# kakao/buffalo

Measured on NVIDIA H100. Metric: interactions/sec (nnz/s) ALS d=128, higher is better.
Workload: dtype f32

## Files before the change

buffalo_b200/csrc/als_tc.cuh:

```cuda
#pragma once
#include "als_generic.cuh"
#include "bfl_common.cuh"
#include <type_traits>

#include "sm90_ptx.cuh"

namespace bfl {
namespace tc {

using namespace sm90;

constexpr int N_CONV = 4, KH = N_CONV / 4;
constexpr int W_EPI = 0, W_MMA = 4, W_CONV = 8, W_PLAN = W_CONV + N_CONV;
constexpr int WARPS = 16, THREADS = WARPS * 32;
constexpr int REG_MMA = 200, REG_PLAN = 4 * 128 - 128 - 128 - REG_MMA;
constexpr int NXS = 8;
constexpr int PT = 2;
constexpr int NR = 2;
constexpr int NO = 2;
constexpr int GATHER_AHEAD = 1;
constexpr int NPG = 8, NP = NPG * PT;
constexpr int NBV = 8;
template <int D>
struct Cfg {
    static constexpr int TILE = D == 128 ? 32 : 16;
    static constexpr int NF = D / 128;
    static constexpr int LBO = D * 16;
    static constexpr int OP_BYTES = TILE * D * 2;
};
constexpr uint32_t F_FIRST = 1u << 8, F_LAST = 1u << 9, F_NEG = 1u << 10, F_STOP = 1u << 11;

__device__ __forceinline__ int msw(int c) { return ((c >> 1) & 3) << 3; }

template <int D>
struct Smem {
    static constexpr int TILE = Cfg<D>::TILE;
    alignas(1024) unsigned char op[NO][PT][2][Cfg<D>::OP_BYTES];
    alignas(128) float raw[NR][PT][TILE * D];
    alignas(128) float mat[128 * 128];
    alignas(16) float bvec[NBV][KH][D];
    alignas(16) float sumq[NBV][KH][D];
    alignas(16) float xs[NXS][D];
    alignas(16) float pv[4][32];
    alignas(16) float dl[4][32];
    alignas(16) float sws[NP][TILE];
    alignas(16) float wv[NP][TILE];
    alignas(16) int32_t keys[NP][TILE];
    float wsum[NBV][KH];
    uint32_t meta_raw[NP];
    uint32_t meta_op[NO][PT];
    int badrow[NXS];
    alignas(8) uint64_t plan_full[NPG], plan_empty[NPG], raw_full[NR], raw_empty[NR], op_full[NO], op_empty[NO];
    alignas(8) uint64_t acc_full, acc_empty, x_full[NXS], d_full[4];
};

struct TcArgs {
    AlsArgs a;
    const int32_t* items;
    float* scratch;
    int64_t split;
    int pass;
    int debug;
};

template <int D>
__host__ __device__ constexpr size_t scratch_floats() { return (size_t)D * D + 2 * D + 4; }

__global__ void tc_absmax_kernel(const float* __restrict__ p, size_t n, unsigned int* __restrict__ out) {
    float m = 0.f;
    const size_t gtid = (size_t)blockIdx.x * blockDim.x + threadIdx.x, gsz = (size_t)gridDim.x * blockDim.x;
    const size_t lead = min(n, (size_t)(((16 - ((uintptr_t)p & 15)) & 15) / 4));
    const size_t n4 = (n - lead) / 4;
    const float4* p4 = reinterpret_cast<const float4*>(p + lead);
    for (size_t i = gtid; i < n4; i += gsz) {
        const float4 v = __ldg(p4 + i);
        m = fmaxf(fmaxf(m, fmaxf(fabsf(v.x), fabsf(v.y))), fmaxf(fabsf(v.z), fabsf(v.w)));
    }
    for (size_t i = gtid; i < lead; i += gsz) m = fmaxf(m, fabsf(p[i]));
    for (size_t i = lead + n4 * 4 + gtid; i < n; i += gsz) m = fmaxf(m, fabsf(p[i]));
    for (int o = 16; o > 0; o >>= 1) m = fmaxf(m, __shfl_xor_sync(FULL, m, o));
    if ((threadIdx.x & 31) == 0 && m > 0.f) atomicMax(out, __float_as_uint(m));
}
__global__ void tc_scale_kernel(const unsigned int* __restrict__ ymax, const unsigned int* __restrict__ vmax, float alpha,
                                float* __restrict__ out) {
    const float y = __uint_as_float(*ymax), w = __uint_as_float(*vmax) * fabsf(alpha);
    const float top = y * sqrtf(w);
    int e = 0;
    if (top > 0.f && isfinite(top)) {
        int ex;
        frexpf(top, &ex);
        e = 15 - ex;
    }
    e = max(-60, min(60, e));
    out[0] = ldexpf(1.f, e);
    out[1] = ldexpf(1.f, -2 * e);
}

template <int D, bool PARTIAL, bool LOSS1>
__global__ void __launch_bounds__(THREADS, 1) als_tc_kernel(TcArgs ta) {
    static_assert(D == 128 || (D == 256 && PARTIAL), "fused row solve: d = 128; split-row mode: d = 128 or 256");
    constexpr int TILE = Cfg<D>::TILE, NF = Cfg<D>::NF, LBO = Cfg<D>::LBO;
    extern __shared__ __align__(1024) unsigned char smem_raw_[];
    Smem<D>& S = *reinterpret_cast<Smem<D>*>(smem_raw_);
    const AlsArgs& a = ta.a;
    const int tid = threadIdx.x, lane = tid & 31;
    const int warp = __shfl_sync(FULL, tid >> 5, 0);

    if (tid == 0) {
        for (int i = 0; i < NR; ++i) {
            mbar_init(&S.raw_full[i], N_CONV);
            mbar_init(&S.raw_empty[i], N_CONV);
        }
        for (int i = 0; i < NPG; ++i) {
            mbar_init(&S.plan_full[i], 1);
            mbar_init(&S.plan_empty[i], N_CONV);
        }
        for (int i = 0; i < NO; ++i) {
            mbar_init(&S.op_full[i], N_CONV);
            mbar_init(&S.op_empty[i], 4);
        }
        mbar_init(&S.acc_full, 4);
        mbar_init(&S.acc_empty, 4);
        for (int b = 0; b < 4; ++b) mbar_init(&S.d_full[b], 1);
        for (int i = 0; i < NXS; ++i) {
            mbar_init(&S.x_full[i], 4);
            S.badrow[i] = 0;
        }
        mbar_init_fence();
    }
    __syncthreads();
    const float scale = __ldg(a.tc_scales), inv2 = __ldg(a.tc_scales + 1);

    const int64_t nitems = a.row_end - a.row_begin;
    const int64_t my_first = (int64_t)blockIdx.x;
    const int64_t stride = gridDim.x;

    auto item_info = [&](int64_t it, int& row, int64_t& beg, int64_t& n, int& slot) {
        if (PARTIAL) {
            const int32_t* p = ta.items + 3 * (a.row_begin + it);
            row = p[0];
            const int64_t rb = row == 0 ? 0 : a.indptr[row - 1];
            const int64_t rn = a.indptr[row] - rb;
            beg = rb + (int64_t)p[1] * ta.split;
            n = min(ta.split, rn - (int64_t)p[1] * ta.split);
            slot = p[2];
        } else {
            row = a.row_list[a.row_begin + it];
            beg = row == 0 ? 0 : a.indptr[row - 1];
            n = a.indptr[row] - beg;
            slot = 0;
        }
    };

    if (warp >= W_PLAN) {
        setmaxnreg_dec<REG_PLAN>();
        if (warp != W_PLAN) return;
        uint32_t gsl = 0, rph = 0, pe = 0;
        auto tile_begin = [&]() -> uint32_t {
            if (pe == 0) mbar_wait_idle(&S.plan_empty[gsl], rph ^ 1u);
            return gsl * PT + pe;
        };
        auto tile_end = [&]() {
            if (++pe == PT) {
                if (lane == 0) mbar_arrive(&S.plan_full[gsl]);
                pe = 0;
                if (++gsl == NPG) { gsl = 0; rph ^= 1u; }
            }
        };
        auto emit = [&](unsigned mask, uint32_t flags, int32_t key, float w) {
            const int cnt = __popc(mask);
            const int slot = __popc(mask & ((1u << lane) - 1u));
            const uint32_t rs = tile_begin();
            if ((mask >> lane) & 1u) {
                S.keys[rs][slot] = key;
                S.sws[rs][slot] = sqrtf(fabsf(w)) * scale;
                S.wv[rs][slot] = w;
            } else {
                const int zslot = cnt + lane - slot;
                if (zslot < TILE) {
                    S.sws[rs][zslot] = 0.f;
                    S.wv[rs][zslot] = 0.f;
                }
            }
            if (lane == 0) S.meta_raw[rs] = (uint32_t)cnt | flags;
            __syncwarp();
            tile_end();
        };
        constexpr int SC = 4, SCN = SC * TILE;
        const bool inl = lane < TILE;
        auto load_id = [&](int64_t it, int& row, int& chunk) {
            row = -1;
            chunk = 0;
            if (it < nitems) {
                if (PARTIAL) {
                    const int32_t* p = ta.items + 3 * (a.row_begin + it);
                    row = p[0];
                    chunk = p[1];
                } else {
                    row = a.row_list[a.row_begin + it];
                }
            }
        };
        auto load_span = [&](int row, int chunk, const int32_t*& kp, const float*& vp, int& n) {
            kp = a.keys;
            vp = a.vals;
            n = 0;
            if (row >= 0) {
                const int64_t rb = row == 0 ? 0 : a.indptr[row - 1];
                const int64_t rn = a.indptr[row] - rb;
                int64_t beg = rb;
                n = (int)rn;
                if (PARTIAL) {
                    beg = rb + (int64_t)chunk * ta.split;
                    n = (int)min(ta.split, rn - (int64_t)chunk * ta.split);
                }
                kp = a.keys + (beg - a.shift);
                vp = a.vals + (beg - a.shift);
            }
        };
        auto load_sc = [&](const int32_t* kp, const float* vp, int n, int c0, int32_t (&key)[SC], float (&w)[SC]) {
#pragma unroll
            for (int s = 0; s < SC; ++s) {
                const int idx = c0 + s * TILE + lane;
                const bool ok = inl && idx < n;
                key[s] = ok ? kp[idx] : 0;
                w[s] = ok ? vp[idx] * a.alpha : 0.f;
            }
        };
        auto emit_sc = [&](int n, int c0, const int32_t (&key)[SC], const float (&w)[SC]) {
            bool neg = false;
#pragma unroll
            for (int s = 0; s < SC; ++s) neg |= w[s] < 0.f;
            if (!__any_sync(FULL, neg)) {
#pragma unroll
                for (int s = 0; s < SC; ++s) {
                    const int t0 = c0 + s * TILE;
                    if (t0 < n) {
                        const uint32_t meta = (uint32_t)min(TILE, n - t0) | (t0 == 0 ? F_FIRST : 0u) | (t0 + TILE >= n ? F_LAST : 0u);
                        const uint32_t rs = tile_begin();
                        if (inl) {
                            float sq;
                            asm("sqrt.approx.ftz.f32 %0, %1;" : "=f"(sq) : "f"(w[s]));
                            S.keys[rs][lane] = key[s];
                            S.sws[rs][lane] = sq * scale;
                            S.wv[rs][lane] = w[s];
                        }
                        if (lane == 0) S.meta_raw[rs] = meta;
                        __syncwarp();
                        tile_end();
                    }
                }
            } else {
#pragma unroll
                for (int s = 0; s < SC; ++s) {
                    const int t0 = c0 + s * TILE;
                    if (t0 < n) {
                        const bool valid = inl && t0 + lane < n;
                        const unsigned pm = __ballot_sync(FULL, valid && !(w[s] < 0.f));
                        const unsigned nm = __ballot_sync(FULL, valid && (w[s] < 0.f));
                        const bool lastc = t0 + TILE >= n;
                        uint32_t fl = (t0 == 0 ? F_FIRST : 0u);
                        if (pm) {
                            emit(pm, fl | ((lastc && !nm) ? F_LAST : 0u), key[s], w[s]);
                            fl = 0u;
                        }
                        if (nm) emit(nm, fl | F_NEG | (lastc ? F_LAST : 0u), key[s], w[s]);
                    }
                }
            }
        };
        const int32_t *kp0, *kp1, *kp2, *kp3;
        const float *vp0, *vp1, *vp2, *vp3;
        int n0, n1, n2, n3;
        int row_t, ch_t, row4, ch4;
        int32_t k0[SC], k1[SC], k2[SC], nk[SC];
        float w0[SC], w1[SC], w2[SC], nw[SC];
        load_id(my_first, row_t, ch_t);
        load_span(row_t, ch_t, kp0, vp0, n0);
        load_sc(kp0, vp0, n0, 0, k0, w0);
        load_id(my_first + stride, row_t, ch_t);
        load_span(row_t, ch_t, kp1, vp1, n1);
        load_sc(kp1, vp1, n1, 0, k1, w1);
        load_id(my_first + 2 * stride, row_t, ch_t);
        load_span(row_t, ch_t, kp2, vp2, n2);
        load_id(my_first + 3 * stride, row4, ch4);
        for (int64_t it = my_first; it < nitems; it += stride) {
            load_sc(kp2, vp2, n2, 0, k2, w2);
            load_span(row4, ch4, kp3, vp3, n3);
            load_id(it + 4 * stride, row4, ch4);
            for (int c0 = 0; c0 < n0; c0 += SCN) {
                const bool more = c0 + SCN < n0;
                if (more) load_sc(kp0, vp0, n0, c0 + SCN, nk, nw);
                emit_sc(n0, c0, k0, w0);
                if (more) {
#pragma unroll
                    for (int s = 0; s < SC; ++s) { k0[s] = nk[s]; w0[s] = nw[s]; }
                }
            }
#pragma unroll
            for (int s = 0; s < SC; ++s) { k0[s] = k1[s]; w0[s] = w1[s]; k1[s] = k2[s]; w1[s] = w2[s]; }
            kp0 = kp1; vp0 = vp1; n0 = n1; kp1 = kp2; vp1 = vp2; n1 = n2; kp2 = kp3; vp2 = vp3; n2 = n3;
        }
        do {
            const uint32_t rs = tile_begin();
            if (lane == 0) S.meta_raw[rs] = F_STOP;
            __syncwarp();
            tile_end();
        } while (pe != 0);
    } else if (warp >= W_MMA && warp < W_MMA + 4) {
        setmaxnreg_inc<REG_MMA>();
        const int r0 = (D == 256 && ta.pass == 2) ? 128 : 0, c0 = (D == 256 && ta.pass > 0) ? 128 : 0;
        const int wq = warp - W_MMA;
        const int fr = 16 * wq + (lane >> 2), fc = 2 * (lane & 3);
        float d0[64], d1[64];
        auto acc_init = [&]() {
            const float s2 = scale * scale;
#pragma unroll
            for (int n = 0; n < 16; ++n)
#pragma unroll
                for (int h = 0; h < 2; ++h) {
                    const int r = fr + 8 * h, c = 8 * n + fc;
                    float2 g0 = make_float2(0.f, 0.f), g1 = make_float2(0.f, 0.f);
                    if (!PARTIAL) {
                        g0 = __ldg(reinterpret_cast<const float2*>(a.G + (size_t)r * D + c));
                        g1 = __ldg(reinterpret_cast<const float2*>(a.G + (size_t)(r + 64) * D + c));
                        g0.x += r == c ? a.reg : 0.f;
                        g0.y += r == c + 1 ? a.reg : 0.f;
                        g1.x += r + 64 == c ? a.reg : 0.f;
                        g1.y += r + 64 == c + 1 ? a.reg : 0.f;
                    }
                    d0[4 * n + 2 * h] = g0.x * s2; d0[4 * n + 2 * h + 1] = g0.y * s2;
                    d1[4 * n + 2 * h] = g1.x * s2; d1[4 * n + 2 * h + 1] = g1.y * s2;
                }
        };
        uint32_t os = 0, oph = 0, aph = 0;
        int64_t seq = 0;
        bool stop = false;
        acc_init();
        while (!stop) {
            mbar_wait(&S.op_full[os], oph);
            fence_proxy_async_smem();
#pragma unroll 1
            for (int e = 0; e < PT; ++e) {
                const uint32_t meta = S.meta_op[os][e];
                if (meta & F_STOP) {
                    stop = true;
                    break;
                }
                const int ksteps = (ta.debug & 2) ? 0 : (int)(meta & 0xffu);
                const uint32_t hi = s32(&S.op[os][e][0][0]), lo = s32(&S.op[os][e][1][0]);
                wgmma_fence();
#pragma unroll 1
                for (int ks = 0; ks < ksteps; ++ks) {
                    const uint32_t k0 = ks * 2 * LBO;
                    const uint64_t ah0 = smem_desc(hi + k0 + r0 * 16, LBO, 128), ah1 = smem_desc(hi + k0 + (r0 + 64) * 16, LBO, 128);
                    const uint64_t al0 = smem_desc(lo + k0 + r0 * 16, LBO, 128), al1 = smem_desc(lo + k0 + (r0 + 64) * 16, LBO, 128);
                    const uint64_t bh = smem_desc(hi + k0 + c0 * 16, LBO, 128), bl = smem_desc(lo + k0 + c0 * 16, LBO, 128);
                    if (meta & F_NEG) {
                        wgmma_m64n128k16_f16<true>(d0, ah0, bh);
                        wgmma_m64n128k16_f16<true>(d0, ah0, bl);
                        wgmma_m64n128k16_f16<true>(d0, al0, bh);
                        wgmma_m64n128k16_f16<true>(d1, ah1, bh);
                        wgmma_m64n128k16_f16<true>(d1, ah1, bl);
                        wgmma_m64n128k16_f16<true>(d1, al1, bh);
                    } else {
                        wgmma_m64n128k16_f16<false>(d0, ah0, bh);
                        wgmma_m64n128k16_f16<false>(d0, ah0, bl);
                        wgmma_m64n128k16_f16<false>(d0, al0, bh);
                        wgmma_m64n128k16_f16<false>(d1, ah1, bh);
                        wgmma_m64n128k16_f16<false>(d1, ah1, bl);
                        wgmma_m64n128k16_f16<false>(d1, al1, bh);
                    }
                }
                wgmma_commit();
                if (meta & F_LAST) {
                    wgmma_wait<0>();
#pragma unroll
                    for (int i = 0; i < 64; ++i) { acc_fence(d0[i]); acc_fence(d1[i]); }
                    mbar_wait_idle(&S.acc_empty, aph ^ 1u);
                    if (PARTIAL) {
                        const int slot = ta.items[3 * (a.row_begin + my_first + seq * stride) + 2];
                        float* sc = ta.scratch + (size_t)slot * scratch_floats<D>();
#pragma unroll
                        for (int n = 0; n < 16; ++n)
#pragma unroll
                            for (int h = 0; h < 2; ++h)
#pragma unroll
                                for (int i = 0; i < 2; ++i) {
                                    const int r = r0 + fr + 8 * h, c = c0 + 8 * n + fc + i;
                                    const float v0 = d0[4 * n + 2 * h + i] * inv2, v1 = d1[4 * n + 2 * h + i] * inv2;
                                    atomicAdd(sc + (size_t)r * D + c, v0);
                                    atomicAdd(sc + (size_t)(r + 64) * D + c, v1);
                                    if (r0 != c0) {
                                        atomicAdd(sc + (size_t)c * D + r, v0);
                                        atomicAdd(sc + (size_t)c * D + r + 64, v1);
                                    }
                                }
                    } else {
#pragma unroll
                        for (int n = 0; n < 16; ++n)
#pragma unroll
                            for (int h = 0; h < 2; ++h)
#pragma unroll
                                for (int i = 0; i < 2; ++i) {
                                    const int r = fr + 8 * h, c = 8 * n + fc + i;
                                    S.mat[c * 128 + (r ^ msw(c))] = d0[4 * n + 2 * h + i] * inv2;
                                    S.mat[c * 128 + ((r + 64) ^ msw(c))] = d1[4 * n + 2 * h + i] * inv2;
                                }
                    }
                    __syncwarp();
                    if (lane == 0) mbar_arrive(&S.acc_full);
                    aph ^= 1u;
                    ++seq;
                    acc_init();
                }
            }
            wgmma_wait<0>();
#pragma unroll
            for (int i = 0; i < 64; ++i) { acc_fence(d0[i]); acc_fence(d1[i]); }
            __syncwarp();
            if (lane == 0) mbar_arrive(&S.op_empty[os]);
            if (++os == NO) { os = 0; oph ^= 1u; }
        }
    } else if (warp >= W_CONV && warp < W_CONV + N_CONV) {
        const int cta = tid - W_CONV * 32;
        const int ct = cta & 127;
        const int kh = cta >> 7;
        constexpr int CHS = TILE / 8 / KH;
        uint32_t rs = 0, rph = 0, os = 0, oph = 0, bslot = 0;
        float2 bacc[NF], qacc[NF];
        float wacc = 0.f;
#pragma unroll
        for (int f = 0; f < NF; ++f) { bacc[f] = make_float2(0.f, 0.f); qacc[f] = make_float2(0.f, 0.f); }
        const int cw = cta >> 5;
        uint32_t gs = 0, gph = 0, grs = 0, grph = 0;
        bool plan_end = false;
        auto gather = [&]() {
            if (plan_end) {
                cp_async_commit();
                return;
            }
            mbar_wait(&S.plan_full[gs], gph);
            mbar_wait(&S.raw_empty[grs], grph ^ 1u);
            const uint32_t gm0 = S.meta_raw[gs * PT], gm1 = S.meta_raw[gs * PT + 1];
            if (PT == 2 && !(ta.debug & 1) && ((gm0 | gm1) & F_STOP) == 0 && (gm0 & 0xffu) == TILE && (gm1 & 0xffu) == TILE) {
                int32_t kk[PT][TILE / N_CONV];
#pragma unroll
                for (int e = 0; e < PT; ++e)
#pragma unroll
                    for (int i = 0; i < TILE / N_CONV; ++i) kk[e][i] = S.keys[gs * PT + e][cw + N_CONV * i];
#pragma unroll
                for (int e = 0; e < PT; ++e)
#pragma unroll
                    for (int i = 0; i < TILE / N_CONV; ++i) {
                        const float* src = a.Y + (int64_t)kk[e][i] * a.ld + lane * 4;
                        float* dst = &S.raw[grs][e][(cw + N_CONV * i) * D + lane * 4];
#pragma unroll
                        for (int c = 0; c < D / 128; ++c) cp_async16_cg(dst + c * 128, src + c * 128);
                    }
            } else
#pragma unroll
            for (int e = 0; e < PT; ++e) {
                const uint32_t gmeta = S.meta_raw[gs * PT + e];
                if (gmeta & F_STOP) {
                    plan_end = true;
                } else {
                    const int gcnt = (ta.debug & 1) ? 0 : (int)(gmeta & 0xffu);
#pragma unroll
                    for (int i = 0; i < TILE / N_CONV; ++i) {
                        const int slot = cw + N_CONV * i;
                        if (slot < gcnt) {
                            const float* src = a.Y + (int64_t)S.keys[gs * PT + e][slot] * a.ld + lane * 4;
                            float* dst = &S.raw[grs][e][slot * D + lane * 4];
#pragma unroll
                            for (int c = 0; c < D / 128; ++c) cp_async16_cg(dst + c * 128, src + c * 128);
                        }
                    }
                }
            }
            cp_async_commit();
            if (++gs == NPG) { gs = 0; gph ^= 1u; }
            if (++grs == NR) { grs = 0; grph ^= 1u; }
        };
        uint32_t cs = 0;
        bool done = false;
        if (ta.debug & 16) {
            uint32_t ph = 0;
            for (;;) {
                mbar_wait(&S.plan_full[cs], ph);
                const bool stop = (S.meta_raw[cs * PT] | S.meta_raw[cs * PT + 1]) & F_STOP;
                __syncwarp();
                if (lane == 0) mbar_arrive(&S.plan_empty[cs]);
                if (stop) break;
                if (++cs == NPG) { cs = 0; ph ^= 1u; }
            }
            if (cta == 0) S.meta_op[0][0] = F_STOP;
            __syncwarp();
            if (lane == 0) mbar_arrive(&S.op_full[0]);
            done = true;
        }
#pragma unroll 1
        for (int i = 0; i < GATHER_AHEAD && !done; ++i) gather();
        while (!done) {
            gather();
            cp_async_wait_group<GATHER_AHEAD>();
            __syncwarp();
            if (lane == 0) mbar_arrive(&S.raw_full[rs]);
            mbar_wait(&S.raw_full[rs], rph);
            float qv[PT][CHS * 8 * NF];
#pragma unroll
            for (int e = 0; e < PT; ++e)
#pragma unroll
                for (int c = 0; c < CHS; ++c)
#pragma unroll
                    for (int i = 0; i < 8; ++i)
#pragma unroll
                        for (int f = 0; f < NF; ++f)
                            qv[e][(c * 8 + i) * NF + f] = S.raw[rs][e][((kh * CHS + c) * 8 + i) * D + ct + 128 * f];
            mbar_wait(&S.op_empty[os], oph ^ 1u);
            const uint32_t cm0 = S.meta_raw[cs * PT], cm1 = S.meta_raw[cs * PT + 1];
            const bool fast2 = PT == 2 && !(ta.debug & 4) && ((cm0 | cm1) & F_STOP) == 0 && (cm0 & 0xffu) == TILE &&
                               (cm1 & 0xffu) == TILE;
            if (fast2) {
#pragma unroll
                for (int e = 0; e < PT; ++e) {
                    const uint32_t meta = e == 0 ? cm0 : cm1;
                    const uint32_t psl = cs * PT + e;
                    const bool first = (meta & F_FIRST) != 0;
#pragma unroll
                    for (int f = 0; f < NF; ++f) {
                        bacc[f].x = first ? 0.f : bacc[f].x; bacc[f].y = first ? 0.f : bacc[f].y;
                        qacc[f].x = first ? 0.f : qacc[f].x; qacc[f].y = first ? 0.f : qacc[f].y;
                    }
                    wacc = first ? 0.f : wacc;
                    unsigned char* hi = &S.op[os][e][0][0];
                    unsigned char* lo = &S.op[os][e][1][0];
#pragma unroll
                    for (int c = 0; c < CHS; ++c) {
                        const int kc = kh * CHS + c, k0 = kc * 8;
                        const float4 sa = *reinterpret_cast<const float4*>(&S.sws[psl][k0]);
                        const float4 sb = *reinterpret_cast<const float4*>(&S.sws[psl][k0 + 4]);
                        const float4 wa = *reinterpret_cast<const float4*>(&S.wv[psl][k0]);
                        const float4 wb = *reinterpret_cast<const float4*>(&S.wv[psl][k0 + 4]);
                        if (LOSS1) wacc += ((wa.x + wa.y) + (wa.z + wa.w)) + ((wb.x + wb.y) + (wb.z + wb.w));
#pragma unroll
                        for (int f = 0; f < NF; ++f) {
                            const int m = ct + 128 * f;
                            const float* q = &qv[e][0];
                            const float2 q01 = make_float2(q[(c * 8 + 0) * NF + f], q[(c * 8 + 1) * NF + f]);
                            const float2 q23 = make_float2(q[(c * 8 + 2) * NF + f], q[(c * 8 + 3) * NF + f]);
                            const float2 q45 = make_float2(q[(c * 8 + 4) * NF + f], q[(c * 8 + 5) * NF + f]);
                            const float2 q67 = make_float2(q[(c * 8 + 6) * NF + f], q[(c * 8 + 7) * NF + f]);
                            uint4 h4, l4;
                            split_f16x2(f2mul(q01, make_float2(sa.x, sa.y)), h4.x, l4.x);
                            split_f16x2(f2mul(q23, make_float2(sa.z, sa.w)), h4.y, l4.y);
                            split_f16x2(f2mul(q45, make_float2(sb.x, sb.y)), h4.z, l4.z);
                            split_f16x2(f2mul(q67, make_float2(sb.z, sb.w)), h4.w, l4.w);
                            const int off = kc * LBO + (m >> 3) * 128 + (m & 7) * 16;
                            *reinterpret_cast<uint4*>(hi + off) = h4;
                            *reinterpret_cast<uint4*>(lo + off) = l4;
                            bacc[f] = f2fma(make_float2(wa.x, wa.y), q01, bacc[f]);
                            bacc[f] = f2fma(make_float2(wa.z, wa.w), q23, bacc[f]);
                            bacc[f] = f2fma(make_float2(wb.x, wb.y), q45, bacc[f]);
                            bacc[f] = f2fma(make_float2(wb.z, wb.w), q67, bacc[f]);
                            if (LOSS1) {
                                qacc[f].x += (q01.x + q23.x) + (q45.x + q67.x);
                                qacc[f].y += (q01.y + q23.y) + (q45.y + q67.y);
                            }
                        }
                    }
#pragma unroll
                    for (int f = 0; f < NF; ++f) {
                        S.bvec[bslot][kh][ct + 128 * f] = bacc[f].x + bacc[f].y;
                        if (LOSS1) S.sumq[bslot][kh][ct + 128 * f] = qacc[f].x + qacc[f].y;
                    }
                    if (LOSS1 && ct == 0) S.wsum[bslot][kh] = wacc;
                    bslot = (bslot + ((meta & F_LAST) ? 1u : 0u)) & (NBV - 1);
                    if (cta == 0) S.meta_op[os][e] = (uint32_t)(TILE / 16) | (meta & (F_FIRST | F_LAST | F_NEG));
                }
            } else
#pragma unroll
            for (int e = 0; e < PT; ++e) {
                if (done) continue;
                const uint32_t psl = cs * PT + e;
                const uint32_t meta = S.meta_raw[psl];
                if (meta & F_STOP) {
                    if (cta == 0) S.meta_op[os][e] = F_STOP;
                    done = true;
                    continue;
                }
                const int cnt = (int)(meta & 0xffu), ksteps = (cnt + 15) >> 4;
                if (meta & F_FIRST) {
#pragma unroll
                    for (int f = 0; f < NF; ++f) { bacc[f] = make_float2(0.f, 0.f); qacc[f] = make_float2(0.f, 0.f); }
                    wacc = 0.f;
                }
                unsigned char* hi = &S.op[os][e][0][0];
                unsigned char* lo = &S.op[os][e][1][0];
                auto chunk = [&](auto guard, const int c) {
                    constexpr bool GUARD = decltype(guard)::value;
                    const int kc = kh * CHS + c, k0 = kc * 8;
                    const float4 sa = *reinterpret_cast<const float4*>(&S.sws[psl][k0]);
                    const float4 sb = *reinterpret_cast<const float4*>(&S.sws[psl][k0 + 4]);
                    const float4 wa = *reinterpret_cast<const float4*>(&S.wv[psl][k0]);
                    const float4 wb = *reinterpret_cast<const float4*>(&S.wv[psl][k0 + 4]);
                    if (LOSS1) wacc += ((wa.x + wa.y) + (wa.z + wa.w)) + ((wb.x + wb.y) + (wb.z + wb.w));
#pragma unroll
                    for (int f = 0; f < NF; ++f) {
                        const int m = ct + 128 * f;
                        float q[8];
#pragma unroll
                        for (int i = 0; i < 8; ++i) q[i] = qv[e][(c * 8 + i) * NF + f];
                        if (GUARD) {
#pragma unroll
                            for (int i = 0; i < 8; ++i) q[i] = (k0 + i < cnt) ? q[i] : 0.f;
                        }
                        const float2 q01 = make_float2(q[0], q[1]), q23 = make_float2(q[2], q[3]);
                        const float2 q45 = make_float2(q[4], q[5]), q67 = make_float2(q[6], q[7]);
                        uint4 h4, l4;
                        split_f16x2(f2mul(q01, make_float2(sa.x, sa.y)), h4.x, l4.x);
                        split_f16x2(f2mul(q23, make_float2(sa.z, sa.w)), h4.y, l4.y);
                        split_f16x2(f2mul(q45, make_float2(sb.x, sb.y)), h4.z, l4.z);
                        split_f16x2(f2mul(q67, make_float2(sb.z, sb.w)), h4.w, l4.w);
                        const int off = kc * LBO + (m >> 3) * 128 + (m & 7) * 16;
                        *reinterpret_cast<uint4*>(hi + off) = h4;
                        *reinterpret_cast<uint4*>(lo + off) = l4;
                        bacc[f] = f2fma(make_float2(wa.x, wa.y), q01, bacc[f]);
                        bacc[f] = f2fma(make_float2(wa.z, wa.w), q23, bacc[f]);
                        bacc[f] = f2fma(make_float2(wb.x, wb.y), q45, bacc[f]);
                        bacc[f] = f2fma(make_float2(wb.z, wb.w), q67, bacc[f]);
                        if (LOSS1) {
                            qacc[f].x += (q[0] + q[2]) + (q[4] + q[6]);
                            qacc[f].y += (q[1] + q[3]) + (q[5] + q[7]);
                        }
                    }
                };
                if (ta.debug & 4) {
                } else if (cnt == TILE) {
#pragma unroll
                    for (int c = 0; c < CHS; ++c) chunk(std::false_type{}, c);
                } else {
#pragma unroll
                    for (int c = 0; c < CHS; ++c)
                        if (kh * CHS + c < 2 * ksteps) chunk(std::true_type{}, c);
                }
                if (meta & F_LAST) {
#pragma unroll
                    for (int f = 0; f < NF; ++f) {
                        S.bvec[bslot][kh][ct + 128 * f] = bacc[f].x + bacc[f].y;
                        if (LOSS1) S.sumq[bslot][kh][ct + 128 * f] = qacc[f].x + qacc[f].y;
                    }
                    if (LOSS1 && ct == 0) S.wsum[bslot][kh] = wacc;
                    bslot = (bslot + 1) & (NBV - 1);
                }
                if (cta == 0) S.meta_op[os][e] = (uint32_t)ksteps | (meta & (F_FIRST | F_LAST | F_NEG));
            }
            __syncwarp();
            if (lane == 0) {
                mbar_arrive(&S.raw_empty[rs]);
                mbar_arrive(&S.plan_empty[cs]);
                mbar_arrive(&S.op_full[os]);
            }
            cs = (cs + 1) & (NPG - 1);
            if (++rs == NR) { rs = 0; rph ^= 1u; }
            if (++os == NO) { os = 0; oph ^= 1u; }
        }
    } else {
        const int q = warp & 3;
        const int j = q * 32 + lane;
        float* pv = S.pv[q];
        double l_nume = 0.0, l_deno = 0.0;
        const float tol = a.tol;
        if constexpr (PARTIAL) {
            int row = 0, slot = 0, nrow = 0, nslot = 0;
            int64_t beg, n = 0, nbeg, nn = 0;
            if (my_first < nitems) item_info(my_first, row, beg, n, slot);
            for (int64_t seq = 0; my_first + seq * stride < nitems; ++seq) {
                const int64_t nit = my_first + (seq + 1) * stride;
                if (nit < nitems) item_info(nit, nrow, nbeg, nn, nslot);
                const uint32_t aph = (uint32_t)(seq & 1);
                const uint32_t bs = (uint32_t)(seq & (NBV - 1));
                mbar_wait_idle(&S.acc_full, aph);
                float* sc = ta.scratch + (size_t)slot * scratch_floats<D>();
                if (ta.pass == 0) {
                    for (int jj = j; jj < D; jj += 128) {
                        atomicAdd(sc + (size_t)D * D + jj, S.bvec[bs][0][jj] + (KH == 2 ? S.bvec[bs][KH - 1][jj] : 0.f));
                        if (LOSS1) atomicAdd(sc + (size_t)D * D + D + jj, S.sumq[bs][0][jj] + (KH == 2 ? S.sumq[bs][KH - 1][jj] : 0.f));
                    }
                    if (LOSS1 && j == 0) atomicAdd(sc + (size_t)D * D + 2 * D, S.wsum[bs][0] + (KH == 2 ? S.wsum[bs][KH - 1] : 0.f));
                }
                __syncwarp();
                if (lane == 0) mbar_arrive(&S.acc_empty);
                row = nrow; slot = nslot; n = nn;
            }
        } else {
            auto row_of = [&](int64_t sq) -> int {
                const int64_t it = my_first + sq * stride;
                return it < nitems ? a.row_list[a.row_begin + it] : -1;
            };
            auto len_of = [&](int row) -> float {
                if (row < 0 || !a.compute_loss) return 0.f;
                return (float)(a.indptr[row] - (row == 0 ? 0 : a.indptr[row - 1]));
            };
            int row = (ta.debug & 16) ? -1 : row_of(0), row1 = row_of(1), row2 = row_of(2);
            float xj = row >= 0 ? a.X[(int64_t)row * a.ld + j] : 0.f;
            float x1 = row1 >= 0 ? a.X[(int64_t)row1 * a.ld + j] : 0.f;
            float nlen = len_of(row), nlen1 = len_of(row1);
            if (row >= 0) {
                S.xs[0][j] = xj;
                __syncwarp();
                if (lane == 0) mbar_arrive(&S.x_full[0]);
            }
            auto mat = [&](int c) -> float { return S.mat[c * 128 + (j ^ msw(c))]; };
            for (int64_t seq = 0; row >= 0; ++seq) {
                const int row3 = row_of(seq + 3);
                const float x2 = row2 >= 0 ? a.X[(int64_t)row2 * a.ld + j] : 0.f;
                const float nlen2 = len_of(row2);
                if (row1 >= 0) {
                    S.xs[(seq + 1) & (NXS - 1)][j] = x1;
                    __syncwarp();
                    if (lane == 0) mbar_arrive(&S.x_full[(seq + 1) & (NXS - 1)]);
                }
                const uint32_t aph = (uint32_t)(seq & 1);
                const uint32_t bs = (uint32_t)(seq & (NBV - 1));
                const uint32_t xsl = (uint32_t)(seq & (NXS - 1));
                const float* xs = S.xs[xsl];
                mbar_wait(&S.x_full[xsl], (uint32_t)((seq / NXS) & 1));
                mbar_wait_idle(&S.acc_full, aph);
                if (ta.debug & 8) {
                    __syncwarp();
                    if (lane == 0) mbar_arrive(&S.acc_empty);
                    row = row1; row1 = row2; row2 = row3;
                    xj = x1; x1 = x2;
                    continue;
                }
                const float bj = S.bvec[bs][0][j] + (KH == 2 ? S.bvec[bs][KH - 1][j] : 0.f);
                float hM = 0.f;
                float md[32];
#pragma unroll
                for (int c = 0; c < D / 32; ++c) {
                    float h0 = 0.f, h1 = 0.f;
#pragma unroll
                    for (int i = 0; i < 32; i += 4) {
                        const float4 x4 = *reinterpret_cast<const float4*>(xs + c * 32 + i);
                        const float m0 = mat(c * 32 + i), m1 = mat(c * 32 + i + 1), m2 = mat(c * 32 + i + 2), m3 = mat(c * 32 + i + 3);
                        h0 = fmaf(m0, x4.x, h0); h1 = fmaf(m1, x4.y, h1);
                        h0 = fmaf(m2, x4.z, h0); h1 = fmaf(m3, x4.w, h1);
                        if (c == q) { md[i] = m0; md[i + 1] = m1; md[i + 2] = m2; md[i + 3] = m3; }
                    }
                    hM += h0 + h1;
                }
                if (a.compute_loss) {
                    const float kappa = a.adaptive_reg ? nlen : 1.0f;
                    double t = (double)(kappa * a.reg * xj * xj);
                    if (a.axis == 1) {
                        t += (double)xj * (double)hM - (double)(a.reg * xj * xj) -
                             2.0 * (double)xj * ((double)bj + (double)S.sumq[bs][0][j] + (KH == 2 ? (double)S.sumq[bs][KH - 1][j] : 0.0));
                        if (j == 0) {
                            const double ws = (double)S.wsum[bs][0] + (KH == 2 ? (double)S.wsum[bs][KH - 1] : 0.0);
                            t += (double)nlen + ws;
                            l_deno += (double)a.Y_rows + ws;
                        }
                    }
                    l_nume += t;
                }
                float h = hM - bj;
#pragma unroll 1
                for (int B = 0; B < q; ++B) {
                    float mv[32];
#pragma unroll
                    for (int i = 0; i < 32; ++i) mv[i] = mat(B * 32 + i);
                    mbar_wait(&S.d_full[B], aph);
                    float u0 = 0.f, u1 = 0.f;
#pragma unroll
                    for (int i = 0; i < 32; i += 4) {
                        const float4 d4 = *reinterpret_cast<const float4*>(&S.dl[B][i]);
                        u0 = fmaf(mv[i], d4.x, u0);
                        u1 = fmaf(mv[i + 1], d4.y, u1);
                        u0 = fmaf(mv[i + 2], d4.z, u0);
                        u1 = fmaf(mv[i + 3], d4.w, u1);
                    }
                    h -= u0 + u1;
                }
                __syncwarp();
                if (lane == 0) mbar_arrive(&S.acc_empty);
                float xv = 0.f;
                {
                    float r = h, p = h;
                    float rsold = warp_sum(r * r);
                    bool act = rsold > tol;
#pragma unroll 1
                    for (int step = 0; step < 3; ++step) {
                        pv[lane] = p;
                        __syncwarp();
                        float a0 = 0.f, a1 = 0.f, a2 = 0.f, a3 = 0.f;
#pragma unroll
                        for (int i = 0; i < 32; i += 4) {
                            const float4 p4 = *reinterpret_cast<const float4*>(pv + i);
                            a0 = fmaf(md[i], p4.x, a0); a1 = fmaf(md[i + 1], p4.y, a1);
                            a2 = fmaf(md[i + 2], p4.z, a2); a3 = fmaf(md[i + 3], p4.w, a3);
                        }
                        __syncwarp();
                        const float Ap = (a0 + a1) + (a2 + a3);
                        const float pAp = warp_sum(p * Ap);
                        const float ss = act ? __fdividef(rsold, pAp) : 0.f;
                        xv = fmaf(ss, p, xv);
                        r = fmaf(-ss, Ap, r);
                        const float rsnew = warp_sum(r * r);
                        act = act && !(rsnew < tol);
                        if (act) p = fmaf(__fdividef(rsnew, rsold), p, r);
                        rsold = act ? rsnew : rsold;
                    }
                }
                float v = xj - xv;
                const bool badw = __any_sync(FULL, !isfinite(v));
                a.X[(int64_t)row * a.ld + j] = v;
                for (int pr = 0; pr < a.n_peer; ++pr) a.peerX[pr][(int64_t)row * a.ld + j] = v;
                if (q < 3) {
                    S.dl[q][lane] = xv;
                    if (badw && lane == 0) atomicOr(&S.badrow[xsl], 1);
                    __syncwarp();
                    if (lane == 0) mbar_arrive(&S.d_full[q]);
                }
                if (q == 3) {
                    const bool bad = badw || (S.badrow[xsl] != 0);
                    if (bad) {
#pragma unroll
                        for (int c = 0; c < 4; ++c) {
                            a.X[(int64_t)row * a.ld + c * 32 + lane] = 0.f;
                            for (int pr = 0; pr < a.n_peer; ++pr) a.peerX[pr][(int64_t)row * a.ld + c * 32 + lane] = 0.f;
                        }
                        __syncwarp();
                        if (lane == 0) S.badrow[xsl] = 0;
                    }
                }
                row = row1; row1 = row2; row2 = row3;
                xj = x1; x1 = x2;
                nlen = nlen1; nlen1 = nlen2;
            }
            if (a.loss && a.compute_loss) {
                l_nume = warp_sum_d(l_nume);
                l_deno = warp_sum_d(l_deno);
                if (lane == 0 && (l_nume != 0.0 || l_deno != 0.0)) {
                    atomicAdd(a.loss, l_nume);
                    atomicAdd(a.loss + 1, l_deno);
                }
            }
        }
    }
}

inline bool tc_applicable(int optimizer_code, int d, int vdim, int block_size) {
    return optimizer_code == 8 && d == 128 && vdim == 128 && block_size == 32;
}
inline bool tc_split_applicable(int optimizer_code, int d, int vdim, int block_size) {
    return optimizer_code == 8 && (d == 128 || d == 256) && vdim == d && block_size == 32;
}

inline int tc_note_absmax(const float* p, size_t n, unsigned int* out, int num_sms, cudaStream_t st) {
    BFL_CUDA(cudaMemsetAsync(out, 0, sizeof(unsigned int), st));
    if (n == 0) return BFL_OK;
    const int grid = (int)std::min<size_t>((n / 4 + 255) / 256 + 1, (size_t)num_sms * 8);
    tc_absmax_kernel<<<grid, 256, 0, st>>>(p, n, out);
    BFL_LAUNCHED();
    return BFL_OK;
}
inline int tc_update_scale(const unsigned int* ymax, const unsigned int* vmax, float alpha, float* scales, cudaStream_t st) {
    tc_scale_kernel<<<1, 1, 0, st>>>(ymax, vmax, alpha, scales);
    BFL_LAUNCHED();
    return BFL_OK;
}

__global__ void tc_count_items_kernel(const int64_t* __restrict__ indptr, const int32_t* __restrict__ list, int64_t nrows,
                                      int64_t split, unsigned long long* total) {
    for (int64_t i = (int64_t)blockIdx.x * blockDim.x + threadIdx.x; i < nrows; i += (int64_t)gridDim.x * blockDim.x) {
        const int row = list[i];
        const int64_t n = indptr[row] - (row == 0 ? 0 : indptr[row - 1]);
        atomicAdd(total, (unsigned long long)((n + split - 1) / split));
    }
}
__global__ void tc_fill_items_kernel(const int64_t* __restrict__ indptr, const int32_t* __restrict__ list, int64_t nrows,
                                     int64_t split, unsigned long long* cursor, int32_t* __restrict__ items) {
    for (int64_t i = (int64_t)blockIdx.x * blockDim.x + threadIdx.x; i < nrows; i += (int64_t)gridDim.x * blockDim.x) {
        const int row = list[i];
        const int64_t n = indptr[row] - (row == 0 ? 0 : indptr[row - 1]);
        const int64_t nc = (n + split - 1) / split;
        const unsigned long long pos = atomicAdd(cursor, (unsigned long long)nc);
        for (int64_t c = 0; c < nc; ++c) {
            items[3 * (pos + c) + 0] = row;
            items[3 * (pos + c) + 1] = (int32_t)c;
            items[3 * (pos + c) + 2] = (int32_t)i;
        }
    }
}

template <int D>
int tc_launch_partial(const AlsArgs& a, const int32_t* items, int64_t nitems, float* scratch, int64_t nslots,
                      int64_t split, int num_sms, cudaStream_t st) {
    if (nitems <= 0) return BFL_OK;
    if (!a.tc_scales) BFL_FAIL(BFL_ERR_STATE, "tensor-core ALS kernel: operand scale not prepared");
    TcArgs ta;
    ta.a = a;
    ta.a.row_begin = 0;
    ta.a.row_end = nitems;
    ta.items = items;
    ta.scratch = scratch;
    ta.split = split;
    ta.debug = 0;
    BFL_CUDA(cudaMemsetAsync(scratch, 0, sizeof(float) * scratch_floats<D>() * (size_t)nslots, st));
    const size_t smem = sizeof(Smem<D>);
    const int grid = (int)std::min<int64_t>(nitems, (int64_t)num_sms);
    for (ta.pass = 0; ta.pass < (D == 128 ? 1 : 3); ++ta.pass) {
        if (a.compute_loss && a.axis == 1) {
            BFL_CUDA(cudaFuncSetAttribute(als_tc_kernel<D, true, true>, cudaFuncAttributeMaxDynamicSharedMemorySize, (int)smem));
            als_tc_kernel<D, true, true><<<grid, THREADS, smem, st>>>(ta);
        } else {
            BFL_CUDA(cudaFuncSetAttribute(als_tc_kernel<D, true, false>, cudaFuncAttributeMaxDynamicSharedMemorySize, (int)smem));
            als_tc_kernel<D, true, false><<<grid, THREADS, smem, st>>>(ta);
        }
        BFL_LAUNCHED();
    }
    return BFL_OK;
}

inline int tc_launch(const AlsArgs& a, int num_sms, cudaStream_t st) {
    const int64_t nrows = a.row_end - a.row_begin;
    if (nrows <= 0) return BFL_OK;
    if (!a.tc_scales) BFL_FAIL(BFL_ERR_STATE, "tensor-core ALS kernel: operand scale not prepared");
    TcArgs ta;
    ta.a = a;
    ta.items = nullptr;
    ta.scratch = nullptr;
    ta.split = 0;
    ta.pass = 0;
    ta.debug = getenv("BFL_TC_DEBUG") ? atoi(getenv("BFL_TC_DEBUG")) : 0;
    const size_t smem = sizeof(Smem<128>);
    const int grid = (int)std::min<int64_t>(nrows, (int64_t)num_sms);
    if (a.compute_loss && a.axis == 1) {
        BFL_CUDA(cudaFuncSetAttribute(als_tc_kernel<128, false, true>, cudaFuncAttributeMaxDynamicSharedMemorySize, (int)smem));
        als_tc_kernel<128, false, true><<<grid, THREADS, smem, st>>>(ta);
    } else {
        BFL_CUDA(cudaFuncSetAttribute(als_tc_kernel<128, false, false>, cudaFuncAttributeMaxDynamicSharedMemorySize, (int)smem));
        als_tc_kernel<128, false, false><<<grid, THREADS, smem, st>>>(ta);
    }
    BFL_LAUNCHED();
    return BFL_OK;
}

}
}
```

buffalo_b200/csrc/sm90_ptx.cuh:

```cuda
#pragma once
#include <cuda_runtime.h>
#include <stdint.h>

namespace bfl {
namespace sm90 {

__device__ __forceinline__ uint32_t s32(const void* p) { return (uint32_t)__cvta_generic_to_shared(p); }

__device__ __forceinline__ void mbar_init(uint64_t* bar, uint32_t count) {
    asm volatile("mbarrier.init.shared::cta.b64 [%0], %1;" ::"r"(s32(bar)), "r"(count) : "memory");
}
__device__ __forceinline__ void mbar_init_fence() { asm volatile("fence.mbarrier_init.release.cluster;" ::: "memory"); }
__device__ __forceinline__ void mbar_arrive(uint64_t* bar) {
    asm volatile("mbarrier.arrive.shared::cta.b64 _, [%0];" ::"r"(s32(bar)) : "memory");
}
__device__ __forceinline__ bool mbar_try_wait(uint64_t* bar, uint32_t parity) {
    uint32_t ok;
    asm volatile(
        "{\n\t.reg .pred p;\n\t"
        "mbarrier.try_wait.parity.shared::cta.b64 p, [%1], %2;\n\t"
        "selp.b32 %0, 1, 0, p;\n\t}"
        : "=r"(ok)
        : "r"(s32(bar)), "r"(parity)
        : "memory");
    return ok != 0;
}
__device__ __forceinline__ void mbar_wait(uint64_t* bar, uint32_t parity) {
    while (!mbar_try_wait(bar, parity)) {
    }
}
__device__ __forceinline__ void mbar_wait_idle(uint64_t* bar, uint32_t parity) {
    while (!mbar_try_wait(bar, parity)) __nanosleep(128);
}

__device__ __forceinline__ void fence_proxy_async_smem() { asm volatile("fence.proxy.async.shared::cta;" ::: "memory"); }

__device__ __forceinline__ void cp_async16_cg(void* smem_dst, const void* gsrc) {
    asm volatile("cp.async.cg.shared.global [%0], [%1], 16;" ::"r"(s32(smem_dst)), "l"(gsrc) : "memory");
}
__device__ __forceinline__ void cp_async_commit() { asm volatile("cp.async.commit_group;" ::: "memory"); }
template <int N>
__device__ __forceinline__ void cp_async_wait_group() { asm volatile("cp.async.wait_group %0;" ::"n"(N) : "memory"); }

__device__ __forceinline__ uint64_t smem_desc(uint32_t saddr, uint32_t lbo_bytes, uint32_t sbo_bytes) {
    return (uint64_t)((saddr >> 4) & 0x3fffu) | ((uint64_t)((lbo_bytes >> 4) & 0x3fffu) << 16) |
           ((uint64_t)((sbo_bytes >> 4) & 0x3fffu) << 32);
}
__device__ __forceinline__ void wgmma_fence() { asm volatile("wgmma.fence.sync.aligned;" ::: "memory"); }
__device__ __forceinline__ void wgmma_commit() { asm volatile("wgmma.commit_group.sync.aligned;" ::: "memory"); }
template <int N>
__device__ __forceinline__ void wgmma_wait() { asm volatile("wgmma.wait_group.sync.aligned %0;" ::"n"(N) : "memory"); }
template <int N>
__device__ __forceinline__ void setmaxnreg_inc() { asm volatile("setmaxnreg.inc.sync.aligned.u32 %0;" ::"n"(N)); }
template <int N>
__device__ __forceinline__ void setmaxnreg_dec() { asm volatile("setmaxnreg.dec.sync.aligned.u32 %0;" ::"n"(N)); }
__device__ __forceinline__ void acc_fence(float& r) { asm volatile("" : "+f"(r)::"memory"); }

#define BFL_WGMMA_ACC64(d)                                                                                              \
    "+f"(d[0]), "+f"(d[1]), "+f"(d[2]), "+f"(d[3]), "+f"(d[4]), "+f"(d[5]), "+f"(d[6]), "+f"(d[7]), "+f"(d[8]),         \
        "+f"(d[9]), "+f"(d[10]), "+f"(d[11]), "+f"(d[12]), "+f"(d[13]), "+f"(d[14]), "+f"(d[15]), "+f"(d[16]),        \
        "+f"(d[17]), "+f"(d[18]), "+f"(d[19]), "+f"(d[20]), "+f"(d[21]), "+f"(d[22]), "+f"(d[23]), "+f"(d[24]),       \
        "+f"(d[25]), "+f"(d[26]), "+f"(d[27]), "+f"(d[28]), "+f"(d[29]), "+f"(d[30]), "+f"(d[31]), "+f"(d[32]),       \
        "+f"(d[33]), "+f"(d[34]), "+f"(d[35]), "+f"(d[36]), "+f"(d[37]), "+f"(d[38]), "+f"(d[39]), "+f"(d[40]),       \
        "+f"(d[41]), "+f"(d[42]), "+f"(d[43]), "+f"(d[44]), "+f"(d[45]), "+f"(d[46]), "+f"(d[47]), "+f"(d[48]),       \
        "+f"(d[49]), "+f"(d[50]), "+f"(d[51]), "+f"(d[52]), "+f"(d[53]), "+f"(d[54]), "+f"(d[55]), "+f"(d[56]),       \
        "+f"(d[57]), "+f"(d[58]), "+f"(d[59]), "+f"(d[60]), "+f"(d[61]), "+f"(d[62]), "+f"(d[63])
#define BFL_WGMMA_REGS64                                                                                                \
    "{%0, %1, %2, %3, %4, %5, %6, %7, %8, %9, %10, %11, %12, %13, %14, %15, %16, %17, %18, %19, %20, %21, %22, %23, "   \
    "%24, %25, %26, %27, %28, %29, %30, %31, %32, %33, %34, %35, %36, %37, %38, %39, %40, %41, %42, %43, %44, %45, %46, " \
    "%47, %48, %49, %50, %51, %52, %53, %54, %55, %56, %57, %58, %59, %60, %61, %62, %63}"
template <bool NEG>
__device__ __forceinline__ void wgmma_m64n128k16_f16(float (&d)[64], uint64_t adesc, uint64_t bdesc) {
    if (NEG) {
        asm volatile("wgmma.mma_async.sync.aligned.m64n128k16.f32.f16.f16 " BFL_WGMMA_REGS64 ", %64, %65, 1, -1, 1, 0, 0;"
                     : BFL_WGMMA_ACC64(d)
                     : "l"(adesc), "l"(bdesc)
                     : "memory");
    } else {
        asm volatile("wgmma.mma_async.sync.aligned.m64n128k16.f32.f16.f16 " BFL_WGMMA_REGS64 ", %64, %65, 1, 1, 1, 0, 0;"
                     : BFL_WGMMA_ACC64(d)
                     : "l"(adesc), "l"(bdesc)
                     : "memory");
    }
}
#undef BFL_WGMMA_ACC64
#undef BFL_WGMMA_REGS64

__device__ __forceinline__ float2 f2mul(float2 a, float2 b) { return make_float2(__fmul_rn(a.x, b.x), __fmul_rn(a.y, b.y)); }
__device__ __forceinline__ float2 f2fma(float2 a, float2 b, float2 c) {
    return make_float2(fmaf(a.x, b.x, c.x), fmaf(a.y, b.y, c.y));
}
__device__ __forceinline__ void split_f16x2(float2 s, uint32_t& head, uint32_t& tail) {
    float2 h;
    h.x = __uint_as_float(__float_as_uint(s.x) & 0xffffe000u);
    h.y = __uint_as_float(__float_as_uint(s.y) & 0xffffe000u);
    const float2 t = f2fma(h, make_float2(-1.f, -1.f), s);
    asm("cvt.rn.f16x2.f32 %0, %1, %2;" : "=r"(head) : "f"(h.y), "f"(h.x));
    asm("cvt.rn.f16x2.f32 %0, %1, %2;" : "=r"(tail) : "f"(t.y), "f"(t.x));
}

}
}
```

Before: 1.009 billion.

## Exploit Gram symmetry: compute only lower-left block of upper half with m64n64 WGMMA

In the non-partial path, the top 64 rows of the 128x128 Gram accumulation now use m64n64 WGMMA covering only columns 0-63, since the upper-right block mirrors the lower-left block already produced by the d1 accumulator. The epilogue writes the missing block by transposing d1 values into S.mat. This removes about a quarter of the tensor-core work and frees 32 accumulator registers per thread. In exchange the epilogue does extra shared-memory stores, and the result now relies on the accumulated matrix being exactly symmetric.

```diff
diff --git a/buffalo_b200/csrc/als_tc.cuh b/buffalo_b200/csrc/als_tc.cuh
--- a/buffalo_b200/csrc/als_tc.cuh
+++ b/buffalo_b200/csrc/als_tc.cuh
@@ -312,7 +312,8 @@
         const int r0 = (D == 256 && ta.pass == 2) ? 128 : 0, c0 = (D == 256 && ta.pass > 0) ? 128 : 0;
         const int wq = warp - W_MMA;
         const int fr = 16 * wq + (lane >> 2), fc = 2 * (lane & 3);
-        float d0[64], d1[64];
+        constexpr int N0 = PARTIAL ? 16 : 8;
+        float d0[4 * N0], d1[64];
         auto acc_init = [&]() {
             const float s2 = scale * scale;
 #pragma unroll
@@ -322,14 +323,14 @@
                     const int r = fr + 8 * h, c = 8 * n + fc;
                     float2 g0 = make_float2(0.f, 0.f), g1 = make_float2(0.f, 0.f);
                     if (!PARTIAL) {
-                        g0 = __ldg(reinterpret_cast<const float2*>(a.G + (size_t)r * D + c));
+                        if (n < N0) g0 = __ldg(reinterpret_cast<const float2*>(a.G + (size_t)r * D + c));
                         g1 = __ldg(reinterpret_cast<const float2*>(a.G + (size_t)(r + 64) * D + c));
                         g0.x += r == c ? a.reg : 0.f;
                         g0.y += r == c + 1 ? a.reg : 0.f;
                         g1.x += r + 64 == c ? a.reg : 0.f;
                         g1.y += r + 64 == c + 1 ? a.reg : 0.f;
                     }
-                    d0[4 * n + 2 * h] = g0.x * s2; d0[4 * n + 2 * h + 1] = g0.y * s2;
+                    if (n < N0) { d0[4 * n + 2 * h] = g0.x * s2; d0[4 * n + 2 * h + 1] = g0.y * s2; }
                     d1[4 * n + 2 * h] = g1.x * s2; d1[4 * n + 2 * h + 1] = g1.y * s2;
                 }
         };
@@ -357,16 +358,28 @@
                     const uint64_t al0 = smem_desc(lo + k0 + r0 * 16, LBO, 128), al1 = smem_desc(lo + k0 + (r0 + 64) * 16, LBO, 128);
                     const uint64_t bh = smem_desc(hi + k0 + c0 * 16, LBO, 128), bl = smem_desc(lo + k0 + c0 * 16, LBO, 128);
                     if (meta & F_NEG) {
-                        wgmma_m64n128k16_f16<true>(d0, ah0, bh);
-                        wgmma_m64n128k16_f16<true>(d0, ah0, bl);
-                        wgmma_m64n128k16_f16<true>(d0, al0, bh);
+                        if constexpr (PARTIAL) {
+                            wgmma_m64n128k16_f16<true>(d0, ah0, bh);
+                            wgmma_m64n128k16_f16<true>(d0, ah0, bl);
+                            wgmma_m64n128k16_f16<true>(d0, al0, bh);
+                        } else {
+                            wgmma_m64n64k16_f16<true>(d0, ah0, bh);
+                            wgmma_m64n64k16_f16<true>(d0, ah0, bl);
+                            wgmma_m64n64k16_f16<true>(d0, al0, bh);
+                        }
                         wgmma_m64n128k16_f16<true>(d1, ah1, bh);
                         wgmma_m64n128k16_f16<true>(d1, ah1, bl);
                         wgmma_m64n128k16_f16<true>(d1, al1, bh);
                     } else {
-                        wgmma_m64n128k16_f16<false>(d0, ah0, bh);
-                        wgmma_m64n128k16_f16<false>(d0, ah0, bl);
-                        wgmma_m64n128k16_f16<false>(d0, al0, bh);
+                        if constexpr (PARTIAL) {
+                            wgmma_m64n128k16_f16<false>(d0, ah0, bh);
+                            wgmma_m64n128k16_f16<false>(d0, ah0, bl);
+                            wgmma_m64n128k16_f16<false>(d0, al0, bh);
+                        } else {
+                            wgmma_m64n64k16_f16<false>(d0, ah0, bh);
+                            wgmma_m64n64k16_f16<false>(d0, ah0, bl);
+                            wgmma_m64n64k16_f16<false>(d0, al0, bh);
+                        }
                         wgmma_m64n128k16_f16<false>(d1, ah1, bh);
                         wgmma_m64n128k16_f16<false>(d1, ah1, bl);
                         wgmma_m64n128k16_f16<false>(d1, al1, bh);
@@ -376,9 +389,12 @@
                 if (meta & F_LAST) {
                     wgmma_wait<0>();
 #pragma unroll
-                    for (int i = 0; i < 64; ++i) { acc_fence(d0[i]); acc_fence(d1[i]); }
+                    for (int i = 0; i < 64; ++i) {
+                        if (i < 4 * N0) acc_fence(d0[i]);
+                        acc_fence(d1[i]);
+                    }
                     mbar_wait_idle(&S.acc_empty, aph ^ 1u);
-                    if (PARTIAL) {
+                    if constexpr (PARTIAL) {
                         const int slot = ta.items[3 * (a.row_begin + my_first + seq * stride) + 2];
                         float* sc = ta.scratch + (size_t)slot * scratch_floats<D>();
 #pragma unroll
@@ -404,8 +420,12 @@
 #pragma unroll
                                 for (int i = 0; i < 2; ++i) {
                                     const int r = fr + 8 * h, c = 8 * n + fc + i;
-                                    S.mat[c * 128 + (r ^ msw(c))] = d0[4 * n + 2 * h + i] * inv2;
-                                    S.mat[c * 128 + ((r + 64) ^ msw(c))] = d1[4 * n + 2 * h + i] * inv2;
+                                    const float v1 = d1[4 * n + 2 * h + i] * inv2;
+                                    if (n < N0) {
+                                        S.mat[c * 128 + (r ^ msw(c))] = d0[4 * n + 2 * h + i] * inv2;
+                                        S.mat[(r + 64) * 128 + (c ^ msw(r + 64))] = v1;
+                                    }
+                                    S.mat[c * 128 + ((r + 64) ^ msw(c))] = v1;
                                 }
                     }
                     __syncwarp();
@@ -417,7 +437,10 @@
             }
             wgmma_wait<0>();
 #pragma unroll
-            for (int i = 0; i < 64; ++i) { acc_fence(d0[i]); acc_fence(d1[i]); }
+            for (int i = 0; i < 64; ++i) {
+                if (i < 4 * N0) acc_fence(d0[i]);
+                acc_fence(d1[i]);
+            }
             __syncwarp();
             if (lane == 0) mbar_arrive(&S.op_empty[os]);
             if (++os == NO) { os = 0; oph ^= 1u; }
diff --git a/buffalo_b200/csrc/sm90_ptx.cuh b/buffalo_b200/csrc/sm90_ptx.cuh
--- a/buffalo_b200/csrc/sm90_ptx.cuh
+++ b/buffalo_b200/csrc/sm90_ptx.cuh
@@ -83,8 +83,33 @@
                      : "memory");
     }
 }
+#define BFL_WGMMA_ACC32(d)                                                                                              \
+    "+f"(d[0]), "+f"(d[1]), "+f"(d[2]), "+f"(d[3]), "+f"(d[4]), "+f"(d[5]), "+f"(d[6]), "+f"(d[7]), "+f"(d[8]),         \
+        "+f"(d[9]), "+f"(d[10]), "+f"(d[11]), "+f"(d[12]), "+f"(d[13]), "+f"(d[14]), "+f"(d[15]), "+f"(d[16]),        \
+        "+f"(d[17]), "+f"(d[18]), "+f"(d[19]), "+f"(d[20]), "+f"(d[21]), "+f"(d[22]), "+f"(d[23]), "+f"(d[24]),       \
+        "+f"(d[25]), "+f"(d[26]), "+f"(d[27]), "+f"(d[28]), "+f"(d[29]), "+f"(d[30]), "+f"(d[31])
+#define BFL_WGMMA_REGS32                                                                                                \
+    "{%0, %1, %2, %3, %4, %5, %6, %7, %8, %9, %10, %11, %12, %13, %14, %15, %16, %17, %18, %19, %20, %21, %22, %23, "   \
+    "%24, %25, %26, %27, %28, %29, %30, %31}"
+template <bool NEG, int N>
+__device__ __forceinline__ void wgmma_m64n64k16_f16(float (&d)[N], uint64_t adesc, uint64_t bdesc) {
+    static_assert(N >= 32, "m64n64 accumulator: 32 registers");
+    if (NEG) {
+        asm volatile("wgmma.mma_async.sync.aligned.m64n64k16.f32.f16.f16 " BFL_WGMMA_REGS32 ", %32, %33, 1, -1, 1, 0, 0;"
+                     : BFL_WGMMA_ACC32(d)
+                     : "l"(adesc), "l"(bdesc)
+                     : "memory");
+    } else {
+        asm volatile("wgmma.mma_async.sync.aligned.m64n64k16.f32.f16.f16 " BFL_WGMMA_REGS32 ", %32, %33, 1, 1, 1, 0, 0;"
+                     : BFL_WGMMA_ACC32(d)
+                     : "l"(adesc), "l"(bdesc)
+                     : "memory");
+    }
+}
 #undef BFL_WGMMA_ACC64
 #undef BFL_WGMMA_REGS64
+#undef BFL_WGMMA_ACC32
+#undef BFL_WGMMA_REGS32
 
 __device__ __forceinline__ float2 f2mul(float2 a, float2 b) { return make_float2(__fmul_rn(a.x, b.x), __fmul_rn(a.y, b.y)); }
 __device__ __forceinline__ float2 f2fma(float2 a, float2 b, float2 c) {
```

After: 1.088 billion (median of 6 runs). +7.8%, better.
